# meuleman/epilogos

Measured on NVIDIA B200. Metric: bins/sec for expected+scores (S2), higher is better.
Workload: dtype int64+f64

## Files before the change

### epilogos_b200/csrc/common.cuh

```cuda
#pragma once
#include <cuda_runtime.h>
#include <cuda.h>
#include <stddef.h>
#include <stdint.h>
#include <stdio.h>
#include <string.h>

#include "../../include/epilogos_b200.h"

namespace epi {

void set_error(const char* fmt, ...);
int check_device();

#define EPI_CUDA(call)                                                                        \
    do {                                                                                      \
        cudaError_t e__ = (call);                                                             \
        if (e__ != cudaSuccess) {                                                             \
            epi::set_error("%s failed at %s:%d: %s", #call, __FILE__, __LINE__,               \
                           cudaGetErrorString(e__));                                          \
            return 1;                                                                         \
        }                                                                                     \
    } while (0)

#define EPI_REQUIRE(cond, ...)                                                                \
    do {                                                                                      \
        if (!(cond)) {                                                                        \
            epi::set_error(__VA_ARGS__);                                                      \
            return 2;                                                                         \
        }                                                                                     \
    } while (0)

int sm_count();
int persistent_grid(int64_t ntiles, int per_sm);

constexpr int S1_TABLE_MAX_WIDTH = 4095;

struct PrepFlags {
    int has_zero;
};

struct K5TcConsts {
    double dg[EPI_MAX_STATES];
    double scale;
    double cst;
    int has_zero;
    uint32_t m1, m8, m16;
    int fbits;
};

struct DeviceWorkspace {
    unsigned long long reduce_slots[64];
    double log2e[EPI_MAX_STATES * EPI_MAX_STATES];
    PrepFlags prep_flags;
    int s3_symmetric;
    alignas(16) uint8_t k5tc_b_image[8 * EPI_MAX_STATES * 128];
    K5TcConsts k5tc_consts;
    alignas(8) double s1_v64[EPI_MAX_STATES * (S1_TABLE_MAX_WIDTH + 1)];
    alignas(8) float s1_v32[EPI_MAX_STATES * (S1_TABLE_MAX_WIDTH + 1)];
    alignas(8) float perm_v32[2][EPI_MAX_STATES * (S1_TABLE_MAX_WIDTH + 1)];
};
static_assert(offsetof(DeviceWorkspace, k5tc_b_image) % 16 == 0, "the B operand image is a bulk-copy source");
static_assert(offsetof(DeviceWorkspace, s1_v64) % 8 == 0 && offsetof(DeviceWorkspace, s1_v32) % 8 == 0,
              "the S1 value tables need 8-byte alignment");

DeviceWorkspace* device_workspace();

typedef CUresult (*tensor_map_encode_fn)(CUtensorMap*, CUtensorMapDataType, cuuint32_t, void*, const cuuint64_t*,
                                         const cuuint64_t*, const cuuint32_t*, const cuuint32_t*,
                                         CUtensorMapInterleave, CUtensorMapSwizzle, CUtensorMapL2promotion,
                                         CUtensorMapFloatOOBfill);
tensor_map_encode_fn get_tensor_map_encode();

int s1_value_table(const float* e, int K, int width, float* v32, double* v64, cudaStream_t st);

int launch_k2_tc(const uint16_t* cnt, int64_t bins, int K, int64_t* n1, int64_t* n2, cudaStream_t st);
int scores_s2_tc(const uint16_t* cnt, int64_t bins, int K, int width, int64_t perms, const float* e, int* zero_flag,
                 float* o32, double* o64, cudaStream_t st);
bool scores_s2_tc_eligible(int width);
int scores_s2_tc_fixed_point(const float* e, int K, int64_t perms, unsigned long long* mfix_dev, int* fbits_host,
                             cudaStream_t st);

#ifdef __CUDACC__

__device__ __forceinline__ uint32_t smem_u32(const void* p) {
    return static_cast<uint32_t>(__cvta_generic_to_shared(p));
}

__device__ __forceinline__ void mbar_init(uint64_t* bar, uint32_t count) {
    asm volatile("mbarrier.init.shared::cta.b64 [%0], %1;" ::"r"(smem_u32(bar)), "r"(count));
}
__device__ __forceinline__ void mbar_fence_init() {
    asm volatile("fence.mbarrier_init.release.cluster;" ::: "memory");
}
__device__ __forceinline__ void mbar_expect_tx(uint64_t* bar, uint32_t bytes) {
    asm volatile("mbarrier.arrive.expect_tx.shared::cta.b64 _, [%0], %1;" ::"r"(smem_u32(bar)), "r"(bytes)
                 : "memory");
}
__device__ __forceinline__ void mbar_arrive(uint64_t* bar) {
    asm volatile("mbarrier.arrive.shared::cta.b64 _, [%0];" ::"r"(smem_u32(bar)) : "memory");
}
__device__ __forceinline__ void mbar_arrive_after(uint64_t* bar, uint32_t dep) {
    asm volatile("mbarrier.arrive.shared::cta.b64 _, [%0];" ::"r"(smem_u32(bar)), "r"(dep) : "memory");
}
__device__ __forceinline__ void mbar_arrive_after(uint64_t* bar, double dep) {
    asm volatile("mbarrier.arrive.shared::cta.b64 _, [%0];" ::"r"(smem_u32(bar)), "d"(dep) : "memory");
}
__device__ __forceinline__ bool mbar_try_wait(uint64_t* bar, uint32_t parity) {
    uint32_t ok;
    asm volatile(
        "{\n\t.reg .pred p;\n\t"
        "mbarrier.try_wait.parity.shared::cta.b64 p, [%1], %2;\n\t"
        "selp.u32 %0, 1, 0, p;\n\t}"
        : "=r"(ok)
        : "r"(smem_u32(bar)), "r"(parity)
        : "memory");
    return ok != 0;
}
__device__ __forceinline__ void mbar_wait(uint64_t* bar, uint32_t parity) {
    while (!mbar_try_wait(bar, parity)) {
    }
}

__device__ __forceinline__ void tma_load_2d(void* smem_dst, const CUtensorMap* map, int32_t c0, int32_t c1,
                                            uint64_t* bar) {
    asm volatile(
        "cp.async.bulk.tensor.2d.shared::cluster.global.tile.mbarrier::complete_tx::bytes [%0], [%1, {%2, %3}], [%4];"
        ::"r"(smem_u32(smem_dst)), "l"(reinterpret_cast<uint64_t>(map)), "r"(c0), "r"(c1), "r"(smem_u32(bar))
        : "memory");
}
__device__ __forceinline__ void bulk_load_1d(void* smem_dst, const void* gsrc, uint32_t bytes, uint64_t* bar) {
    asm volatile("cp.async.bulk.shared::cluster.global.mbarrier::complete_tx::bytes [%0], [%1], %2, [%3];"
                 ::"r"(smem_u32(smem_dst)), "l"(reinterpret_cast<uint64_t>(gsrc)), "r"(bytes), "r"(smem_u32(bar))
                 : "memory");
}
__device__ __forceinline__ void tma_prefetch_desc(const CUtensorMap* map) {
// ... 49 lines not shown
```

### epilogos_b200/csrc/scores.cu

```cuda
#include "common.cuh"

namespace epi {

constexpr int K5_THREADS = 256;
constexpr int K5_WARPS = K5_THREADS / 32;
constexpr int KT_MAX = EPI_MAX_STATES;

__constant__ __align__(16) double c_log2e[KT_MAX * KT_MAX];

__global__ void k5_prepare_kernel(const float* __restrict__ e, int rows, int cols, int kt, double* __restrict__ out,
                                  PrepFlags* flags) {
    __shared__ int zero;
    if (threadIdx.x == 0) zero = 0;
    __syncthreads();
    for (int i = threadIdx.x; i < rows * kt; i += blockDim.x) {
        const int s = i / kt, q = i - s * kt;
        double v = 0.0;
        if (q < cols) {
            const double ev = (double)e[s * cols + q];
            if (ev > 0.0) v = log2(ev);
            else zero = 1;
        }
        out[i] = v;
    }
    __syncthreads();
    if (threadIdx.x == 0) flags->has_zero = zero;
}

__device__ __forceinline__ double kl_direct(double obs, double e) {
    if (e == 0.0 || obs == 0.0) return 0.0;
    return obs * log2(obs / e);
}

struct WarpCountStream {
    const uint16_t* cnt;
    uint16_t* slab[2];
    uint64_t* bar;
    long long bins, ngroups, stride;
    int K, lane, buf;
    uint32_t phase[2];

    __device__ __forceinline__ void issue(long long g, int b) const {
        if (lane == 0 && g < ngroups && bins - g * 32 >= 32) {
            mbar_expect_tx(&bar[b], 64 * K);
            bulk_load_1d(slab[b], cnt + g * 32 * K, 64 * K, &bar[b]);
        }
    }
    __device__ __forceinline__ const uint16_t* acquire(long long g, int nvalid) {
        const int b = buf;
        buf ^= 1;
        issue(g + stride, b ^ 1);
        if (nvalid == 32) {
            mbar_wait(&bar[b], phase[b]);
            phase[b] ^= 1;
        } else {
            const uint16_t* src = cnt + g * 32 * K;
            for (int i = lane; i < nvalid * K; i += 32) slab[b][i] = src[i];
            __syncwarp();
        }
        return slab[b];
    }
};

__device__ __forceinline__ void warp_store_scores(const float* slab, float* __restrict__ dst, int nvalid, int K,
                                                  int lane) {
    __syncwarp();
    if (nvalid == 32) {
        const float4* s4 = reinterpret_cast<const float4*>(slab);
        float4* d4 = reinterpret_cast<float4*>(dst);
        for (int i = lane; i < 8 * K; i += 32) d4[i] = s4[i];
    } else {
        for (int i = lane; i < nvalid * K; i += 32) dst[i] = slab[i];
    }
    __syncwarp();
}

constexpr int S1_SMEM_TABLE_BYTES = 96 * 1024;

__global__ void k5_s1_table_kernel(const float* __restrict__ exp1, int K, int width, float* __restrict__ v32,
                                   double* __restrict__ v64) {
    const int n = K * (width + 1);
    const double dw = (double)width;
    for (int i = blockIdx.x * blockDim.x + threadIdx.x; i < n; i += gridDim.x * blockDim.x) {
        const int s = i / (width + 1), c = i - s * (width + 1);
// ... 16 lines not shown
    float* vts = reinterpret_cast<float*>(bars + K5_WARPS * 2);

    const int tid = threadIdx.x, warp = tid >> 5, lane = tid & 31;
    const int w1 = width + 1;
    if (tid == 0) {
        for (int i = 0; i < K5_WARPS * 2; ++i) mbar_init(&bars[i], 1);
        mbar_fence_init();
    }
    if (SMEM_TABLE)
        for (int i = tid; i < K * w1; i += K5_THREADS) vts[i] = v32g[i];
    __syncthreads();
    const float* vt = SMEM_TABLE ? vts : v32g;
    float* myf = fslab + warp * 32 * K;

    const long long ngroups = (bins + 31) / 32;
    WarpCountStream in{cnt, {cslab + warp * 64 * K, cslab + warp * 64 * K + 32 * K}, bars + warp * 2, bins, ngroups,
                       (long long)gridDim.x * K5_WARPS, K, lane, 0, {0u, 0u}};
    in.issue((long long)blockIdx.x * K5_WARPS + warp, 0);
    for (long long g = (long long)blockIdx.x * K5_WARPS + warp; g < ngroups; g += in.stride) {
        const long long bin0 = g * 32;
        const int nvalid = (int)((bins - bin0) < 32 ? (bins - bin0) : 32);
        const uint16_t* myc = in.acquire(g, nvalid);
        if (lane < nvalid) {
            const uint16_t* row = myc + lane * K;
            for (int s = 0; s < K; ++s) {
                const int c = row[s];
                myf[lane * K + s] = vt[s * w1 + c];
                if (out64 != nullptr) out64[(bin0 + lane) * K + s] = v64g[s * w1 + c];
            }
        }
        if (out32 != nullptr) warp_store_scores(myf, out32 + bin0 * K, nvalid, K, lane);
        else __syncwarp();
    }
}

__global__ void __launch_bounds__(K5_THREADS) k5_s1_direct_kernel(const uint16_t* __restrict__ cnt, long long bins, int K,
                                                                  int width, const float* __restrict__ exp1,
                                                                  float* __restrict__ out32, double* __restrict__ out64) {
    const double dw = (double)width;
    const long long n = bins * K;
    for (long long i = blockIdx.x * (long long)blockDim.x + threadIdx.x; i < n; i += (long long)gridDim.x * blockDim.x) {
        const int s = (int)(i % K);
        const double v = kl_direct((double)cnt[i] / dw, (double)__ldg(exp1 + s));
        if (out32 != nullptr) out32[i] = (float)v;
        if (out64 != nullptr) out64[i] = v;
    }
}

template <int KT>
__global__ void __launch_bounds__(K5_THREADS) k5_s2_kernel(const uint16_t* __restrict__ cnt, long long bins, int K,
                                                           int width, double perms, const float* __restrict__ exp2,
                                                           const PrepFlags* __restrict__ flags, int force_direct,
                                                           float* __restrict__ out32, double* __restrict__ out64) {
    if (force_direct == 2 && !flags->has_zero) return;
    extern __shared__ __align__(128) uint8_t smem_raw[];
    uint16_t* cslab = reinterpret_cast<uint16_t*>(smem_raw);
    float* fslab = reinterpret_cast<float*>(smem_raw + K5_WARPS * 32 * K * 4);
    uint64_t* bars = reinterpret_cast<uint64_t*>(smem_raw + K5_WARPS * 32 * K * 8);

    const int tid = threadIdx.x, warp = tid >> 5, lane = tid & 31;
    if (tid == 0) {
        for (int i = 0; i < K5_WARPS * 2; ++i) mbar_init(&bars[i], 1);
        mbar_fence_init();
    }
    __syncthreads();
    const double lp = log2(perms);
    const double inv_perms = 1.0 / perms;
    const bool direct = force_direct || flags->has_zero;
    float* myf = fslab + warp * 32 * K;

    const long long ngroups = (bins + 31) / 32;
    WarpCountStream in{cnt, {cslab + warp * 64 * K, cslab + warp * 64 * K + 32 * K}, bars + warp * 2, bins, ngroups,
                       (long long)gridDim.x * K5_WARPS, K, lane, 0, {0u, 0u}};
    in.issue((long long)blockIdx.x * K5_WARPS + warp, 0);
    for (long long g = (long long)blockIdx.x * K5_WARPS + warp; g < ngroups; g += in.stride) {
        const long long bin0 = g * 32;
        const int nvalid = (int)((bins - bin0) < 32 ? (bins - bin0) : 32);
        const uint16_t* myc = in.acquire(g, nvalid);
        if (lane < nvalid) {
            const uint16_t* row = myc + lane * K;
            float* orow = myf + lane * K;
            if (direct) {
                for (int q = 0; q < K; ++q) {
                    const long long cq = row[q];
                    double sum = 0.0;
                    if (cq != 0) {
                        for (int s = 0; s < K; ++s) {
                            const long long cs = row[s];
                            const long long prod = (s == q) ? cs * (cs - 1) : cs * cq;
                            if (prod != 0) sum += kl_direct((double)prod / perms, (double)__ldg(exp2 + s * K + q));
                        }
                    }
                    orow[q] = (float)sum;
                    if (out64 != nullptr) out64[(bin0 + lane) * K + q] = sum;
                }
            } else {
                double cd[KT], mc[KT];
                double a = 0.0, w = 0.0;
#pragma unroll
                for (int s = 0; s < KT; ++s) {
                    const int c = s < K ? row[s] : 0;
                    cd[s] = (double)c;
                    const double l = c > 0 ? log2((double)c) : 0.0;
                    a = fma(cd[s], l, a);
                    w += cd[s];
                    mc[s] = 0.0;
                }
                const double2* le2 = reinterpret_cast<const double2*>(c_log2e);
#pragma unroll
                for (int s = 0; s < KT; ++s) {
#pragma unroll
                    for (int q = 0; q < KT; q += 2) {
                        const double2 m = le2[(s * KT + q) >> 1];
                        mc[q] = fma(cd[s], m.x, mc[q]);
                        mc[q + 1] = fma(cd[s], m.y, mc[q + 1]);
                    }
                }
                const double wm1 = w - 1.0;
#pragma unroll
                for (int q = 0; q < KT; ++q) {
                    if (q < K) {
                        const int c = row[q];
                        const int cm = c > 0 ? c - 1 : 0;
                        const double lt = c > 0 ? log2((double)c) : 0.0;
                        const double l1 = cm > 0 ? log2((double)cm) : 0.0;
                        double br = (a - mc[q]) + c_log2e[q * KT + q];
                        br = fma(lt - lp, wm1, br);
                        br = fma(-cd[q], lt, br);
                        br = fma((double)cm, l1, br);
                        const double v = c > 0 ? (cd[q] * inv_perms) * br : 0.0;
                        orow[q] = (float)v;
                        if (out64 != nullptr) out64[(bin0 + lane) * K + q] = v;
                    }
                }
            }
        }
        if (out32 != nullptr) warp_store_scores(myf, out32 + bin0 * K, nvalid, K, lane);
        else __syncwarp();
    }
}

static int prepare_tables(const float* e, int rows, int cols, int kt, cudaStream_t st, const PrepFlags** flags_out) {
    DeviceWorkspace* ws = device_workspace();
    EPI_REQUIRE(ws != nullptr, "could not allocate the per-device workspace");
    k5_prepare_kernel<<<1, 256, 0, st>>>(e, rows, cols, kt, ws->log2e, &ws->prep_flags);
// ... 17 lines not shown
        const int64_t cap = (int64_t)sm_count() * 16;
        if (blocks > cap) blocks = cap;
        k5_s1_direct_kernel<<<(unsigned)blocks, K5_THREADS, 0, st>>>(cnt, bins, K, width, e, o32, o64);
        EPI_CUDA(cudaGetLastError());
        return 0;
    }
    DeviceWorkspace* ws = device_workspace();
    EPI_REQUIRE(ws != nullptr, "could not allocate the per-device workspace");
    double* v64 = ws->s1_v64;
    float* v32 = ws->s1_v32;
    const int n = K * (width + 1);
    if (int rc = s1_value_table(e, K, width, v32, v64, st)) return rc;
    const size_t base = (size_t)K5_WARPS * 32 * K * 8 + K5_WARPS * 16;
    const size_t table = (size_t)n * 4;
    const int64_t ntiles = (bins + K5_THREADS - 1) / K5_THREADS;
    const size_t base_big = (size_t)32 * 32 * K * 8 + 32 * 16;
    if (table <= (size_t)S1_SMEM_TABLE_BYTES && 4 * (base + table + 1024) > (size_t)220 * 1024 &&
        base_big + table + 1024 <= (size_t)226 * 1024) {
        auto kern = k5_s1_kernel<true, 1024>;
        EPI_CUDA(cudaFuncSetAttribute(kern, cudaFuncAttributeMaxDynamicSharedMemorySize, (int)(base_big + table)));
        kern<<<persistent_grid((bins + 1023) / 1024, 1), 1024, base_big + table, st>>>(cnt, bins, K, width, v32, v64, o32, o64);
    } else if (table <= (size_t)S1_SMEM_TABLE_BYTES) {
        auto kern = k5_s1_kernel<true, K5_THREADS>;
        EPI_CUDA(cudaFuncSetAttribute(kern, cudaFuncAttributeMaxDynamicSharedMemorySize, (int)(base + table)));
        const int per_sm = (int)((size_t)220 * 1024 / (base + table + 1024));
        kern<<<persistent_grid(ntiles, per_sm < 1 ? 1 : (per_sm > 4 ? 4 : per_sm)), K5_THREADS, base + table, st>>>(
            cnt, bins, K, width, v32, v64, o32, o64);
    } else {
        auto kern = k5_s1_kernel<false, K5_THREADS>;
        EPI_CUDA(cudaFuncSetAttribute(kern, cudaFuncAttributeMaxDynamicSharedMemorySize, (int)base));
        kern<<<persistent_grid(ntiles, 4), K5_THREADS, base, st>>>(cnt, bins, K, width, v32, v64, o32, o64);
    }
    EPI_CUDA(cudaGetLastError());
    return 0;
}

template <int KT>
static int launch_s2(const uint16_t* cnt, int64_t bins, int K, int width, int64_t perms, const float* e,
                     const PrepFlags* flags, int direct, float* o32, double* o64, cudaStream_t st) {
    auto kern = k5_s2_kernel<KT>;
    const size_t smem = (size_t)K5_WARPS * 32 * K * 8 + K5_WARPS * 16;
    EPI_CUDA(cudaFuncSetAttribute(kern, cudaFuncAttributeMaxDynamicSharedMemorySize, (int)smem));
    const int64_t ntiles = (bins + K5_THREADS - 1) / K5_THREADS;
    kern<<<persistent_grid(ntiles, 3), K5_THREADS, smem, st>>>(cnt, bins, K, width, (double)perms, e, flags, direct, o32,
                                                                o64);
    EPI_CUDA(cudaGetLastError());
    return 0;
}

template <int KT>
static int dispatch_s2(const uint16_t* cnt, int64_t bins, int K, int width, int64_t perms, const float* e, float* o32,
                       double* o64, int mode, cudaStream_t st) {
    const PrepFlags* flags = nullptr;
    if (mode == EPI_SCORE_TABLE && scores_s2_tc_eligible(width)) {
        DeviceWorkspace* ws = device_workspace();
        EPI_REQUIRE(ws != nullptr, "could not allocate the per-device workspace");
        PrepFlags* fl = &ws->prep_flags;
        if (int rc = scores_s2_tc(cnt, bins, K, width, perms, e, &fl->has_zero, o32, o64, st)) return rc;
        return launch_s2<KT>(cnt, bins, K, width, perms, e, fl, 2, o32, o64, st);
    }
    if (int rc = prepare_tables(e, K, K, KT, st, &flags)) return rc;
    return launch_s2<KT>(cnt, bins, K, width, perms, e, flags, mode == EPI_SCORE_DIRECT, o32, o64, st);
}

}

using namespace epi;

static int check_score_args(const void* cnt, int64_t bins, int K, int width, const void* e, int mode) {
    if (check_device()) return 3;
    EPI_REQUIRE(bins >= 0 && bins < (1ll << 31), "bins=%lld out of range", (long long)bins);
    EPI_REQUIRE(K >= 1 && K <= EPI_MAX_STATES, "num_states=%d out of range [1, %d]", K, EPI_MAX_STATES);
    EPI_REQUIRE(width >= 1 && width <= 65535, "width=%d out of range [1, 65535]", width);
    EPI_REQUIRE(mode == EPI_SCORE_TABLE || mode == EPI_SCORE_DIRECT, "unknown score mode %d", mode);
    if (bins == 0) return 0;
    EPI_REQUIRE(cnt != nullptr && e != nullptr, "null pointer argument");
    EPI_REQUIRE((reinterpret_cast<uintptr_t>(cnt) & 15) == 0, "cnt_dev must be 16-byte aligned");
    return 0;
}

extern "C" int epi_scores_s1(const uint16_t* cnt_dev, int64_t bins, int32_t K, int32_t width, const float* exp1_dev,
                             float* out32_dev, double* out64_dev, int32_t mode, void* stream_) {
    cudaStream_t st = static_cast<cudaStream_t>(stream_);
    if (int rc = check_score_args(cnt_dev, bins, K, width, exp1_dev, mode)) return rc;
    if (bins == 0 || (out32_dev == nullptr && out64_dev == nullptr)) return 0;
    EPI_REQUIRE(out32_dev == nullptr || (reinterpret_cast<uintptr_t>(out32_dev) & 15) == 0,
                "out32_dev must be 16-byte aligned");
    return launch_s1(cnt_dev, bins, K, width, exp1_dev, mode == EPI_SCORE_DIRECT, out32_dev, out64_dev, st);
}

extern "C" int epi_scores_s2_fixed_point(const float* exp2_dev, int32_t K, int64_t perms, uint64_t* mfix_dev,
                                         int32_t* fraction_bits_out, void* stream_) {
    cudaStream_t st = static_cast<cudaStream_t>(stream_);
    if (check_device()) return 3;
    EPI_REQUIRE(K >= 1 && K <= EPI_MAX_STATES, "num_states=%d out of range [1, %d]", K, EPI_MAX_STATES);
    EPI_REQUIRE(perms >= 1 && exp2_dev != nullptr && mfix_dev != nullptr, "bad argument");
    int fbits = 0;
    if (int rc = scores_s2_tc_fixed_point(exp2_dev, K, perms, reinterpret_cast<unsigned long long*>(mfix_dev), &fbits, st))
        return rc;
    if (fraction_bits_out) *fraction_bits_out = fbits;
    return 0;
}

extern "C" int epi_scores_s2(const uint16_t* cnt_dev, int64_t bins, int32_t K, int32_t width, int64_t perms,
                             const float* exp2_dev, float* out32_dev, double* out64_dev, int32_t mode, void* stream_) {
    cudaStream_t st = static_cast<cudaStream_t>(stream_);
    if (int rc = check_score_args(cnt_dev, bins, K, width, exp2_dev, mode)) return rc;
    EPI_REQUIRE(perms >= 1, "perms=%lld must be positive (needs at least 2 biosamples)", (long long)perms);
    if (bins == 0 || (out32_dev == nullptr && out64_dev == nullptr)) return 0;
    EPI_REQUIRE(out32_dev == nullptr || (reinterpret_cast<uintptr_t>(out32_dev) & 15) == 0,
                "out32_dev must be 16-byte aligned");
    if (K <= 16) return dispatch_s2<16>(cnt_dev, bins, K, width, perms, exp2_dev, out32_dev, out64_dev, mode, st);
    if (K <= 18) return dispatch_s2<18>(cnt_dev, bins, K, width, perms, exp2_dev, out32_dev, out64_dev, mode, st);
// ... 3 lines not shown
```

### epilogos_b200/csrc/tc_tables.cu

```cuda
#include "common.cuh"
#include "tc05.cuh"
#include "count_tile.cuh"

namespace epi {

constexpr int T2_BINS = 128;
constexpr int T2_STAGES = 4;
constexpr int T2_OPS = 2;
constexpr int T2_THREADS = 192;
constexpr int T2_TMEM_COLS = 128;

template <int KT, int KR>
__global__ void __launch_bounds__(T2_THREADS, 4)
k2_tc_kernel(const uint16_t* __restrict__ cnt, long long bins, int Krt, unsigned long long* __restrict__ n1,
             unsigned long long* __restrict__ n2) {
    const int K = KR ? KR : Krt;
    constexpr int NCOL = ((2 * KT + 1) + 15) & ~15;
    extern __shared__ uint8_t smem_raw[];
    uint8_t* smem = smem_raw + ((1024u - (smem_u32(smem_raw) & 1023u)) & 1023u);
    const int tile_bytes = T2_BINS * K * 2;
    uint8_t* ops = smem;
    uint8_t* ring = ops + T2_OPS * T2_OP_BYTES;
    uint64_t* ld_full = reinterpret_cast<uint64_t*>(ring + T2_STAGES * tile_bytes);
    uint64_t* ld_empty = ld_full + T2_STAGES;
// ... 96 lines not shown
                    drain_gram<NCOL>(tmem_base + ((uint32_t)(warp * 32) << 16), warp, lane, K, n1, n2);
                    tc_fence_before();
                    __syncwarp();
                    if (lane == 0) mbar_arrive(acc_empty);
                }
            }
        }
    }
    tc_fence_before();
    __syncthreads();
    if (warp == 5) tmem_dealloc(tmem_base, T2_TMEM_COLS);
}

template <int KT, int KR>
static int launch_k2_tc_impl(const uint16_t* cnt, int64_t bins, int K, int64_t* n1, int64_t* n2, cudaStream_t st) {
    const size_t smem = 1024 + (size_t)T2_OPS * T2_OP_BYTES + (size_t)T2_STAGES * T2_BINS * K * 2 +
                        (2 * T2_STAGES + 2 * T2_OPS + 2) * 8 + 16;
    auto kern = k2_tc_kernel<KT, KR>;
    EPI_CUDA(cudaFuncSetAttribute(kern, cudaFuncAttributeMaxDynamicSharedMemorySize, (int)smem));
    const int64_t ntiles = (bins + T2_BINS - 1) / T2_BINS;
    const int ctas = 4;
    kern<<<persistent_grid(ntiles, ctas), T2_THREADS, smem, st>>>(cnt, (long long)bins, K,
                                                                reinterpret_cast<unsigned long long*>(n1),
                                                                reinterpret_cast<unsigned long long*>(n2));
    EPI_CUDA(cudaGetLastError());
    return 0;
}

int launch_k2_tc(const uint16_t* cnt, int64_t bins, int K, int64_t* n1, int64_t* n2, cudaStream_t st) {
    if (K == 18) return launch_k2_tc_impl<18, 18>(cnt, bins, K, n1, n2, st);
    if (K == 15) return launch_k2_tc_impl<16, 15>(cnt, bins, K, n1, n2, st);
    if (K <= 16) return launch_k2_tc_impl<16, 0>(cnt, bins, K, n1, n2, st);
    if (K <= 18) return launch_k2_tc_impl<18, 0>(cnt, bins, K, n1, n2, st);
    return launch_k2_tc_impl<32, 0>(cnt, bins, K, n1, n2, st);
}

constexpr int T5_BINS = 128;
constexpr int T5_A_BYTES = 128 * 128;
constexpr unsigned long long T5_MAGIC = 0x4338000000000000ull;
constexpr int T5_MAX_WIDTH = 2047;

__device__ __forceinline__ unsigned long long mad_wide(uint32_t a, uint32_t b, unsigned long long c) {
    unsigned long long d;
    asm("mad.wide.u32 %0, %1, %2, %3;" : "=l"(d) : "r"(a), "r"(b), "l"(c));
    return d;
}

__device__ __forceinline__ uint32_t mad_lo(uint32_t a, uint32_t b, uint32_t c) {
    uint32_t d;
    asm("mad.lo.u32 %0, %1, %2, %3;" : "=r"(d) : "r"(a), "r"(b), "r"(c));
    return d;
}

__constant__ K5TcConsts c_k5tc;

__global__ void k5tc_prepare_kernel(const float* __restrict__ e, int K, double perms, int nrows,
                                    uint8_t* __restrict__ b_image, K5TcConsts* __restrict__ out, int* __restrict__ zero_flag,
                                    unsigned long long* __restrict__ mfix_out) {
    __shared__ unsigned long long mfix[EPI_MAX_STATES * EPI_MAX_STATES];
    __shared__ double mval[EPI_MAX_STATES * EPI_MAX_STATES];
    __shared__ unsigned long long maxbits;
    __shared__ int zero, fbits;
    if (threadIdx.x == 0) {
        maxbits = 0ull;
        zero = 0;
    }
    __syncthreads();
    for (int i = threadIdx.x; i < K * K; i += blockDim.x) {
        const double ev = (double)e[i];
        double m = 0.0;
        if (ev > 0.0) m = -log2(ev);
        else zero = 1;
        if (m < 0.0) m = 0.0;
        mval[i] = m;
        atomicMax(&maxbits, (unsigned long long)__double_as_longlong(m));
    }
    __syncthreads();
    if (threadIdx.x == 0) {
        const double mx = __longlong_as_double((long long)maxbits);
        int ib = 1;
        while (ib < 12 && (double)(1ull << ib) <= mx) ++ib;
        fbits = 56 - ib;
    }
    __syncthreads();
    const int F = fbits;
    for (int i = threadIdx.x; i < K * K; i += blockDim.x) {
        unsigned long long v = (unsigned long long)llrint(ldexp(mval[i], F));
        if (v >= (1ull << 56)) v = (1ull << 56) - 1;
        mfix[i] = v;
        if (mfix_out != nullptr) mfix_out[i] = v;
    }
    for (int i = threadIdx.x; i < nrows * 128 / 4; i += blockDim.x) reinterpret_cast<uint32_t*>(b_image)[i] = 0u;
    __syncthreads();
    for (int i = threadIdx.x; i < K * K * 14; i += blockDim.x) {
        const int dd = i % 7, h = (i / 7) & 1, st = i / 14;
        const int s = st / K, t = st - s * K;
        const uint32_t n = (uint32_t)(t * 8 + dd + h), k = (uint32_t)(2 * s + h);
        b_image[sw128_offset(n, k)] = (uint8_t)((mfix[st] >> (8 * dd)) & 255ull);
    }
    if (threadIdx.x < K) out->dg[threadIdx.x] = ldexp((double)mfix[threadIdx.x * K + threadIdx.x], -F - 3) / perms;
    if (threadIdx.x == 0) {
        const double scale = ldexp(1.0, -F) / perms;
        out->scale = scale;
        out->cst = 6755399441055744.0 * scale;
        out->has_zero = zero;
        out->m1 = 1u;
        out->m8 = 1u << 8;
        out->m16 = 1u << 16;
        out->fbits = F;
        *zero_flag = zero;
    }
}

template <int KT, int KR, int NWG, bool WANT64>
__global__ void __launch_bounds__(NWG * 128 + 64, 1)
k5_s2_tc_kernel(const uint16_t* __restrict__ cnt, long long bins, int Krt, int width, double perms,
                const uint8_t* __restrict__ b_image, float* __restrict__ out32, double* __restrict__ out64) {
    if (c_k5tc.has_zero) return;

    static_assert(KT % 2 == 0, "KT must be even");
    constexpr int NPAD = ((8 * KT + 31) / 32) * 32;
    static_assert(NPAD * NWG <= 512, "accumulator regions exceed TMEM");
    constexpr int KSTEPS = (2 * KT + 31) / 32;
    const int K = KR ? KR : Krt;

    extern __shared__ uint8_t smem_raw[];
    uint8_t* smem = smem_raw + ((1024u - (smem_u32(smem_raw) & 1023u)) & 1023u);
    const int slab_bytes = T5_BINS * K * 2;
    uint8_t* a_ops = smem;
    uint8_t* b_op = a_ops + NWG * T5_A_BYTES;
    uint8_t* slabs = b_op + NPAD * 128;
    float* stage = reinterpret_cast<float*>(slabs + NWG * 2 * slab_bytes);
    double* g1 = reinterpret_cast<double*>(stage + NWG * T5_BINS * K);
    double* f1 = g1 + ((width + 2) & ~1);
    uint64_t* ld_full = reinterpret_cast<uint64_t*>(f1 + ((width + 2) & ~1));
    uint64_t* ld_empty = ld_full + NWG * 2;
    uint64_t* a_full = ld_empty + NWG * 2;
    uint64_t* mma_done = a_full + NWG;
    uint64_t* b_full = mma_done + NWG;
    uint32_t* tmem_slot = reinterpret_cast<uint32_t*>(b_full + 1);

    const int tid = threadIdx.x, warp = tid >> 5, lane = tid & 31;
    constexpr int NT = NWG * 128 + 64;
    const long long ntiles = (bins + T5_BINS - 1) / T5_BINS;
    const long long nfull = bins / T5_BINS;

    for (int i = tid; i < NWG * T5_A_BYTES / 16; i += NT) reinterpret_cast<uint4*>(a_ops)[i] = make_uint4(0u, 0u, 0u, 0u);
    {
        const double lp = log2(perms), invp = 1.0 / perms, wm1 = (double)width - 1.0;
        for (int c = tid; c <= width; c += NT) {
            const double l = c > 0 ? log2((double)c) : 0.0;
            const double l1 = c > 1 ? log2((double)(c - 1)) : 0.0;
            const double cl = (double)c * l;
            f1[c] = cl * invp;
            g1[c] = (double)c * ((fma(l - lp, wm1, -cl) + (double)(c > 0 ? c - 1 : 0) * l1) * invp);
        }
    }
    fence_proxy_async_smem();
    if (tid == 0) {
        for (int i = 0; i < NWG * 2; ++i) {
            mbar_init(&ld_full[i], 1);
            mbar_init(&ld_empty[i], 4);
        }
        for (int g = 0; g < NWG; ++g) {
            mbar_init(&a_full[g], 4);
            mbar_init(&mma_done[g], 1);
        }
        mbar_init(b_full, 1);
        mbar_fence_init();
    }
    if (warp == 4 * NWG + 1) tmem_alloc(tmem_slot, 512);
    tc_fence_before();
    __syncthreads();
    tc_fence_after();
    const uint32_t tmem_base = *tmem_slot;

    if (warp == 4 * NWG) {
        if (lane == 0) {
            mbar_expect_tx(b_full, NPAD * 128);
            bulk_load_1d(b_op, b_image, NPAD * 128, b_full);
            int j = 0;
            for (long long t = blockIdx.x; t < nfull; t += gridDim.x, ++j) {
                const int g = j % NWG, u = j / NWG, b = u & 1;
                mbar_wait_wd(&ld_empty[g * 2 + b], (((uint32_t)(u >> 1)) & 1u) ^ 1u);
                mbar_expect_tx(&ld_full[g * 2 + b], (uint32_t)slab_bytes);
                bulk_load_1d(slabs + (g * 2 + b) * slab_bytes, cnt + t * (long long)T5_BINS * K, (uint32_t)slab_bytes,
                             &ld_full[g * 2 + b]);
            }
        }
    } else if (warp == 4 * NWG + 1) {
        if (lane == 0) {
            const uint32_t nmma = (uint32_t)((8 * K + 15) & ~15);
            const uint32_t idesc = umma_i8_idesc(128, nmma);
            mbar_wait_wd(b_full, 0);
            const uint64_t b_desc = make_kmajor_sw128_desc(smem_u32(b_op));
            int j = 0;
            for (long long t = blockIdx.x; t < ntiles; t += gridDim.x, ++j) {
                const int g = j % NWG, u = j / NWG;
                mbar_wait_spin_wd(&a_full[g], ((uint32_t)u) & 1u);
                tc_fence_after();
                const uint64_t a_desc = make_kmajor_sw128_desc(smem_u32(a_ops + g * T5_A_BYTES));
#pragma unroll
                for (int k = 0; k < KSTEPS; ++k)
                    umma_i8(tmem_base + (uint32_t)(g * NPAD), a_desc + 2 * k, b_desc + 2 * k, idesc, k ? 1u : 0u);
                umma_commit(&mma_done[g]);
            }
        }
    } else {
        const int g = warp >> 2, r = tid & 127;
        uint8_t* a_row = a_ops + g * T5_A_BYTES + r * 128;
        float* mystage = stage + g * T5_BINS * K;
        const uint32_t taddr = tmem_base + ((uint32_t)((warp & 3) * 32) << 16) + (uint32_t)(g * NPAD);
        const double scale = c_k5tc.scale * 0.125, cst = c_k5tc.cst, scale32 = c_k5tc.scale * (4294967296.0 * 0.125);
        int u = 0;
        for (long long t = blockIdx.x + (long long)g * gridDim.x; t < ntiles; t += (long long)NWG * gridDim.x, ++u) {
            const long long bin0 = t * T5_BINS;
            const int b = u & 1;
            uint32_t cw[KT / 2];
            if (t < nfull) {
                mbar_wait_wd(&ld_full[g * 2 + b], ((uint32_t)(u >> 1)) & 1u);
                load_count_row<KT, KR>(reinterpret_cast<const uint16_t*>(slabs + (g * 2 + b) * slab_bytes) + r * K, K, cw);
            } else {
                load_count_row_guarded<KT>(cnt + (bin0 + r) * K, K, bin0 + r < bins, cw);
            }
            store_operand_row<KT>(a_row, r, cw, -1, 0u);
            fence_proxy_async_smem();
            __syncwarp();
            if (lane == 0) {
                mbar_arrive(&a_full[g]);
                if (t < nfull) mbar_arrive(&ld_empty[g * 2 + b]);
            }

            uint32_t co[KT];
#pragma unroll
            for (int s = 0; s < KT; ++s) co[s] = ((cw[s >> 1] >> (16 * (s & 1))) & 0xffffu) << 3;
            double a4[4] = {0.0, 0.0, 0.0, 0.0};
#pragma unroll
            for (int s = 0; s < KT; ++s) a4[s & 3] += *reinterpret_cast<const double*>(reinterpret_cast<const uint8_t*>(f1) + co[s]);
            const double a_adj = (((a4[0] + a4[1]) + (a4[2] + a4[3])) - cst) * 0.125;

            if (lane == 0) bulk_wait_read0();
            __syncwarp();
            mbar_wait_wd(&mma_done[g], ((uint32_t)u) & 1u);
            tc_fence_after();
#pragma unroll
            for (int c0 = 0; c0 < 8 * KT; c0 += 32) {
                uint32_t v[32];
                double chg[4], cd[4];
#pragma unroll
                for (int i = 0; i < 4; ++i) {
                    const int tt = (c0 / 8 + i < KT) ? c0 / 8 + i : 0;
                    chg[i] = *reinterpret_cast<const double*>(reinterpret_cast<const uint8_t*>(g1) + co[tt]);
                    cd[i] = __hiloint2double(0x43300000, (int)co[tt]) - 4503599627370496.0;
                }
                tmem_ld_32x32(taddr + (uint32_t)c0, v);
                float f[4];
#pragma unroll
                for (int i = 0; i < 4; ++i) {
                    const int tt = c0 / 8 + i;
                    f[i] = 0.0f;
                    if (tt < KT && (KR == 0 || tt < KR)) {
                        const uint32_t t01 = mad_lo(v[8 * i + 1], c_k5tc.m8, v[8 * i]);
                        const uint32_t t23 = mad_lo(v[8 * i + 3], c_k5tc.m8, v[8 * i + 2]);
                        const uint32_t t45 = mad_lo(v[8 * i + 5], c_k5tc.m8, v[8 * i + 4]);
                        const uint32_t t67 = mad_lo(v[8 * i + 7], c_k5tc.m8, v[8 * i + 6]);
                        const unsigned long long lb = mad_wide(t23, c_k5tc.m16, ((unsigned long long)(T5_MAGIC >> 32) << 32) | t01);
                        const unsigned long long hb = mad_wide(t67, c_k5tc.m16, ((unsigned long long)(T5_MAGIC >> 32) << 32) | t45);
                        const double dl = __longlong_as_double((long long)lb);
                        const double dh = __longlong_as_double((long long)hb) - 6755399441055744.0;
                        const double base = fma(dh, scale32, fma(dl, scale, a_adj)) - c_k5tc.dg[tt];
                        const double val = fma(cd[i], base, chg[i]);
                        f[i] = (float)val;
                        if (WANT64 && (KR != 0 || tt < K) && bin0 + r < bins) out64[(bin0 + r) * K + tt] = val;
                    }
                }
                if constexpr (KR != 0 && KR % 2 == 0) {
                    float2* dst = reinterpret_cast<float2*>(mystage + r * KR + c0 / 8);
                    if (c0 / 8 < KR) dst[0] = make_float2(f[0], f[1]);
                    if (c0 / 8 + 2 < KR) dst[1] = make_float2(f[2], f[3]);
                } else {
#pragma unroll
                    for (int i = 0; i < 4; ++i)
                        if (c0 / 8 + i < K) mystage[r * K + c0 / 8 + i] = f[i];
                }
            }
            tc_fence_before();
            fence_proxy_async_smem();
            __syncwarp();
            if (out32 != nullptr) {
                const int wq = warp & 3;
                const long long wbin0 = bin0 + 32 * wq;
                if (t < nfull) {
                    if (lane == 0) {
                        bulk_store_1d(out32 + wbin0 * K, mystage + 32 * wq * K, (uint32_t)(32 * K * 4));
                        bulk_commit();
                    }
                } else if (wbin0 < bins) {
                    const int n = (int)((bins - wbin0) < 32 ? (bins - wbin0) : 32) * K;
                    for (int i = lane; i < n; i += 32) out32[wbin0 * K + i] = mystage[32 * wq * K + i];
                }
            }
        }
        if (lane == 0) bulk_wait0();
    }
    tc_fence_before();
    __syncthreads();
    if (warp == 4 * NWG + 1) tmem_dealloc(tmem_base, 512);
}

template <int KT, int KR, int NWG, bool WANT64>
static int launch_k5_tc2(const uint16_t* cnt, int64_t bins, int K, int width, int64_t perms, const uint8_t* b_image,
                         float* o32, double* o64, cudaStream_t st) {
    constexpr int NPAD = ((8 * KT + 31) / 32) * 32;
    auto kern = k5_s2_tc_kernel<KT, KR, NWG, WANT64>;
    const size_t smem = 1024 + (size_t)NWG * T5_A_BYTES + (size_t)NPAD * 128 + (size_t)NWG * 2 * T5_BINS * K * 2 +
                        (size_t)NWG * T5_BINS * K * 4 + (size_t)(width + 2) * 16 +
                        (size_t)(6 * NWG + 1) * 8 + 16;
    EPI_CUDA(cudaFuncSetAttribute(kern, cudaFuncAttributeMaxDynamicSharedMemorySize, (int)smem));
    const int64_t ntiles = (bins + T5_BINS - 1) / T5_BINS;
    kern<<<persistent_grid(ntiles, 1), NWG * 128 + 64, smem, st>>>(cnt, (long long)bins, K, width, (double)perms, b_image,
                                                                    o32, o64);
    EPI_CUDA(cudaGetLastError());
    return 0;
}

template <int KT, int KR, int NWG>
static int launch_k5_tc(const uint16_t* cnt, int64_t bins, int K, int width, int64_t perms, const float* e, int* zero_flag,
                        float* o32, double* o64, cudaStream_t st) {
    constexpr int NPAD = ((8 * KT + 31) / 32) * 32;
    static_assert(NPAD * 128 <= sizeof(DeviceWorkspace::k5tc_b_image), "B operand image exceeds its workspace region");
    DeviceWorkspace* ws = device_workspace();
    EPI_REQUIRE(ws != nullptr, "could not allocate the per-device workspace");
    k5tc_prepare_kernel<<<1, 256, 0, st>>>(e, K, (double)perms, NPAD, ws->k5tc_b_image, &ws->k5tc_consts, zero_flag, nullptr);
    EPI_CUDA(cudaGetLastError());
    EPI_CUDA(cudaMemcpyToSymbolAsync(c_k5tc, &ws->k5tc_consts, sizeof(K5TcConsts), 0, cudaMemcpyDeviceToDevice, st));
    if (o64 != nullptr) return launch_k5_tc2<KT, KR, NWG, true>(cnt, bins, K, width, perms, ws->k5tc_b_image, o32, o64, st);
    return launch_k5_tc2<KT, KR, NWG, false>(cnt, bins, K, width, perms, ws->k5tc_b_image, o32, o64, st);
}

int scores_s2_tc(const uint16_t* cnt, int64_t bins, int K, int width, int64_t perms, const float* e, int* zero_flag,
                 float* o32, double* o64, cudaStream_t st) {
    if (K == 18) return launch_k5_tc<18, 18, 3>(cnt, bins, K, width, perms, e, zero_flag, o32, o64, st);
    if (K == 15) return launch_k5_tc<16, 15, 4>(cnt, bins, K, width, perms, e, zero_flag, o32, o64, st);
    if (K <= 16) return launch_k5_tc<16, 0, 4>(cnt, bins, K, width, perms, e, zero_flag, o32, o64, st);
    if (K <= 18) return launch_k5_tc<18, 0, 3>(cnt, bins, K, width, perms, e, zero_flag, o32, o64, st);
    return launch_k5_tc<32, 0, 2>(cnt, bins, K, width, perms, e, zero_flag, o32, o64, st);
}

bool scores_s2_tc_eligible(int width) { return width <= T5_MAX_WIDTH; }

int scores_s2_tc_fixed_point(const float* e, int K, int64_t perms, unsigned long long* mfix_dev, int* fbits_host,
                             cudaStream_t st) {
    DeviceWorkspace* ws = device_workspace();
    EPI_REQUIRE(ws != nullptr, "could not allocate the per-device workspace");
    k5tc_prepare_kernel<<<1, 256, 0, st>>>(e, K, (double)perms, 8 * EPI_MAX_STATES, ws->k5tc_b_image, &ws->k5tc_consts,
                                           &ws->prep_flags.has_zero, mfix_dev);
    EPI_CUDA(cudaGetLastError());
    K5TcConsts host;
    EPI_CUDA(cudaMemcpyAsync(&host, &ws->k5tc_consts, sizeof(host), cudaMemcpyDeviceToHost, st));
    EPI_CUDA(cudaStreamSynchronize(st));
    if (fbits_host) *fbits_host = host.fbits;
    return 0;
}

}
```

Measured before the change: 5.263 billion.

## Fold zero-fallback into TC kernel, decouple TMEM accumulators from warpgroups

Removes the constant-memory copy and the separate fallback launch: the TC scoring kernel now reads the constants through a pointer and handles the has-zero case itself with an inline direct-score loop. TMEM accumulator regions are decoupled from warpgroups through NACC slots guarded by acc_empty barriers. This allows K=18 to run 4 warpgroups with 3 accumulators. The intent is fewer launches and memcpys per call and more epilogue warpgroups for K in 17–18, at the cost of extra barrier waits, and the MMA can stall until an accumulator is freed.

Measured after the change: 5.351 billion, median of 6. +1.7%, better.

```diff
diff --git a/epilogos_b200/csrc/common.cuh b/epilogos_b200/csrc/common.cuh
--- a/epilogos_b200/csrc/common.cuh
+++ b/epilogos_b200/csrc/common.cuh
@@ -45,7 +45,6 @@
     double scale;
     double cst;
     int has_zero;
-    uint32_t m1, m8, m16;
     int fbits;
 };
 
@@ -75,13 +74,31 @@
 int s1_value_table(const float* e, int K, int width, float* v32, double* v64, cudaStream_t st);
 
 int launch_k2_tc(const uint16_t* cnt, int64_t bins, int K, int64_t* n1, int64_t* n2, cudaStream_t st);
-int scores_s2_tc(const uint16_t* cnt, int64_t bins, int K, int width, int64_t perms, const float* e, int* zero_flag,
-                 float* o32, double* o64, cudaStream_t st);
+int scores_s2_tc(const uint16_t* cnt, int64_t bins, int K, int width, int64_t perms, const float* e, float* o32,
+                 double* o64, cudaStream_t st);
 bool scores_s2_tc_eligible(int width);
 int scores_s2_tc_fixed_point(const float* e, int K, int64_t perms, unsigned long long* mfix_dev, int* fbits_host,
                              cudaStream_t st);
 
 #ifdef __CUDACC__
+
+__device__ __forceinline__ double kl_direct(double obs, double e) {
+    if (e == 0.0 || obs == 0.0) return 0.0;
+    return obs * log2(obs / e);
+}
+__device__ __forceinline__ double s2_direct_score(const uint16_t* row, int K, int q, double perms,
+                                                  const float* __restrict__ exp2) {
+    const long long cq = row[q];
+    double sum = 0.0;
+    if (cq != 0) {
+        for (int s = 0; s < K; ++s) {
+            const long long cs = row[s];
+            const long long prod = (s == q) ? cs * (cs - 1) : cs * cq;
+            if (prod != 0) sum += kl_direct((double)prod / perms, (double)__ldg(exp2 + s * K + q));
+        }
+    }
+    return sum;
+}
 
 __device__ __forceinline__ uint32_t smem_u32(const void* p) {
     return static_cast<uint32_t>(__cvta_generic_to_shared(p));
diff --git a/epilogos_b200/csrc/scores.cu b/epilogos_b200/csrc/scores.cu
--- a/epilogos_b200/csrc/scores.cu
+++ b/epilogos_b200/csrc/scores.cu
@@ -25,11 +25,6 @@
     }
     __syncthreads();
     if (threadIdx.x == 0) flags->has_zero = zero;
-}
-
-__device__ __forceinline__ double kl_direct(double obs, double e) {
-    if (e == 0.0 || obs == 0.0) return 0.0;
-    return obs * log2(obs / e);
 }
 
 struct WarpCountStream {
@@ -152,7 +147,6 @@
                                                            int width, double perms, const float* __restrict__ exp2,
                                                            const PrepFlags* __restrict__ flags, int force_direct,
                                                            float* __restrict__ out32, double* __restrict__ out64) {
-    if (force_direct == 2 && !flags->has_zero) return;
     extern __shared__ __align__(128) uint8_t smem_raw[];
     uint16_t* cslab = reinterpret_cast<uint16_t*>(smem_raw);
     float* fslab = reinterpret_cast<float*>(smem_raw + K5_WARPS * 32 * K * 4);
@@ -182,15 +176,7 @@
             float* orow = myf + lane * K;
             if (direct) {
                 for (int q = 0; q < K; ++q) {
-                    const long long cq = row[q];
-                    double sum = 0.0;
-                    if (cq != 0) {
-                        for (int s = 0; s < K; ++s) {
-                            const long long cs = row[s];
-                            const long long prod = (s == q) ? cs * (cs - 1) : cs * cq;
-                            if (prod != 0) sum += kl_direct((double)prod / perms, (double)__ldg(exp2 + s * K + q));
-                        }
-                    }
+                    const double sum = s2_direct_score(row, K, q, perms, exp2);
                     orow[q] = (float)sum;
                     if (out64 != nullptr) out64[(bin0 + lane) * K + q] = sum;
                 }
@@ -314,13 +300,8 @@
 static int dispatch_s2(const uint16_t* cnt, int64_t bins, int K, int width, int64_t perms, const float* e, float* o32,
                        double* o64, int mode, cudaStream_t st) {
     const PrepFlags* flags = nullptr;
-    if (mode == EPI_SCORE_TABLE && scores_s2_tc_eligible(width)) {
-        DeviceWorkspace* ws = device_workspace();
-        EPI_REQUIRE(ws != nullptr, "could not allocate the per-device workspace");
-        PrepFlags* fl = &ws->prep_flags;
-        if (int rc = scores_s2_tc(cnt, bins, K, width, perms, e, &fl->has_zero, o32, o64, st)) return rc;
-        return launch_s2<KT>(cnt, bins, K, width, perms, e, fl, 2, o32, o64, st);
-    }
+    if (mode == EPI_SCORE_TABLE && scores_s2_tc_eligible(width))
+        return scores_s2_tc(cnt, bins, K, width, perms, e, o32, o64, st);
     if (int rc = prepare_tables(e, K, K, KT, st, &flags)) return rc;
     return launch_s2<KT>(cnt, bins, K, width, perms, e, flags, mode == EPI_SCORE_DIRECT, o32, o64, st);
 }
diff --git a/epilogos_b200/csrc/tc_tables.cu b/epilogos_b200/csrc/tc_tables.cu
--- a/epilogos_b200/csrc/tc_tables.cu
+++ b/epilogos_b200/csrc/tc_tables.cu
@@ -172,10 +172,10 @@
     return d;
 }
 
-__constant__ K5TcConsts c_k5tc;
+__constant__ uint32_t c_m8 = 1u << 8, c_m16 = 1u << 16;
 
 __global__ void k5tc_prepare_kernel(const float* __restrict__ e, int K, double perms, int nrows,
-                                    uint8_t* __restrict__ b_image, K5TcConsts* __restrict__ out, int* __restrict__ zero_flag,
+                                    uint8_t* __restrict__ b_image, K5TcConsts* __restrict__ out,
                                     unsigned long long* __restrict__ mfix_out) {
     __shared__ unsigned long long mfix[EPI_MAX_STATES * EPI_MAX_STATES];
     __shared__ double mval[EPI_MAX_STATES * EPI_MAX_STATES];
@@ -218,33 +218,44 @@
         const uint32_t n = (uint32_t)(t * 8 + dd + h), k = (uint32_t)(2 * s + h);
         b_image[sw128_offset(n, k)] = (uint8_t)((mfix[st] >> (8 * dd)) & 255ull);
     }
-    if (threadIdx.x < K) out->dg[threadIdx.x] = ldexp((double)mfix[threadIdx.x * K + threadIdx.x], -F - 3) / perms;
+    if (threadIdx.x < EPI_MAX_STATES)
+        out->dg[threadIdx.x] = threadIdx.x < K ? ldexp((double)mfix[threadIdx.x * K + threadIdx.x], -F - 3) / perms : 0.0;
     if (threadIdx.x == 0) {
         const double scale = ldexp(1.0, -F) / perms;
         out->scale = scale;
         out->cst = 6755399441055744.0 * scale;
         out->has_zero = zero;
-        out->m1 = 1u;
-        out->m8 = 1u << 8;
-        out->m16 = 1u << 16;
         out->fbits = F;
-        *zero_flag = zero;
-    }
-}
-
-template <int KT, int KR, int NWG, bool WANT64>
+    }
+}
+
+template <int KT, int KR, int NWG, int NACC, bool WANT64>
 __global__ void __launch_bounds__(NWG * 128 + 64, 1)
 k5_s2_tc_kernel(const uint16_t* __restrict__ cnt, long long bins, int Krt, int width, double perms,
-                const uint8_t* __restrict__ b_image, float* __restrict__ out32, double* __restrict__ out64) {
-    if (c_k5tc.has_zero) return;
-
+                const uint8_t* __restrict__ b_image, const K5TcConsts* __restrict__ kc, const float* __restrict__ exp2,
+                float* __restrict__ out32, double* __restrict__ out64) {
     static_assert(KT % 2 == 0, "KT must be even");
     constexpr int NPAD = ((8 * KT + 31) / 32) * 32;
-    static_assert(NPAD * NWG <= 512, "accumulator regions exceed TMEM");
+    static_assert(NPAD * NACC <= 512, "accumulator regions exceed TMEM");
+    static_assert(NACC <= NWG, "more accumulator regions than warpgroups to fill them");
     constexpr int KSTEPS = (2 * KT + 31) / 32;
+    constexpr int NT = NWG * 128 + 64;
     const int K = KR ? KR : Krt;
+    const int tid = threadIdx.x, warp = tid >> 5, lane = tid & 31;
+
+    if (kc->has_zero) {
+        const long long n = bins * K;
+        for (long long i = (long long)blockIdx.x * NT + tid; i < n; i += (long long)gridDim.x * NT) {
+            const long long b = i / K;
+            const double v = s2_direct_score(cnt + b * K, K, (int)(i - b * K), perms, exp2);
+            if (out32 != nullptr) out32[i] = (float)v;
+            if (WANT64) out64[i] = v;
+        }
+        return;
+    }
 
     extern __shared__ uint8_t smem_raw[];
+    __shared__ __align__(16) double s_dg[EPI_MAX_STATES];
     uint8_t* smem = smem_raw + ((1024u - (smem_u32(smem_raw) & 1023u)) & 1023u);
     const int slab_bytes = T5_BINS * K * 2;
     uint8_t* a_ops = smem;
@@ -257,15 +268,15 @@
     uint64_t* ld_empty = ld_full + NWG * 2;
     uint64_t* a_full = ld_empty + NWG * 2;
     uint64_t* mma_done = a_full + NWG;
-    uint64_t* b_full = mma_done + NWG;
+    uint64_t* acc_empty = mma_done + NWG;
+    uint64_t* b_full = acc_empty + NACC;
     uint32_t* tmem_slot = reinterpret_cast<uint32_t*>(b_full + 1);
 
-    const int tid = threadIdx.x, warp = tid >> 5, lane = tid & 31;
-    constexpr int NT = NWG * 128 + 64;
     const long long ntiles = (bins + T5_BINS - 1) / T5_BINS;
     const long long nfull = bins / T5_BINS;
 
     for (int i = tid; i < NWG * T5_A_BYTES / 16; i += NT) reinterpret_cast<uint4*>(a_ops)[i] = make_uint4(0u, 0u, 0u, 0u);
+    if (tid < EPI_MAX_STATES) s_dg[tid] = kc->dg[tid];
     {
         const double lp = log2(perms), invp = 1.0 / perms, wm1 = (double)width - 1.0;
         for (int c = tid; c <= width; c += NT) {
@@ -286,6 +297,7 @@
             mbar_init(&a_full[g], 4);
             mbar_init(&mma_done[g], 1);
         }
+        for (int q = 0; q < NACC; ++q) mbar_init(&acc_empty[q], 4);
         mbar_init(b_full, 1);
         mbar_fence_init();
     }
@@ -316,13 +328,14 @@
             const uint64_t b_desc = make_kmajor_sw128_desc(smem_u32(b_op));
             int j = 0;
             for (long long t = blockIdx.x; t < ntiles; t += gridDim.x, ++j) {
-                const int g = j % NWG, u = j / NWG;
+                const int g = j % NWG, u = j / NWG, q = j % NACC, n = j / NACC;
+                mbar_wait_spin_wd(&acc_empty[q], (((uint32_t)n) & 1u) ^ 1u);
                 mbar_wait_spin_wd(&a_full[g], ((uint32_t)u) & 1u);
                 tc_fence_after();
                 const uint64_t a_desc = make_kmajor_sw128_desc(smem_u32(a_ops + g * T5_A_BYTES));
 #pragma unroll
                 for (int k = 0; k < KSTEPS; ++k)
-                    umma_i8(tmem_base + (uint32_t)(g * NPAD), a_desc + 2 * k, b_desc + 2 * k, idesc, k ? 1u : 0u);
+                    umma_i8(tmem_base + (uint32_t)(q * NPAD), a_desc + 2 * k, b_desc + 2 * k, idesc, k ? 1u : 0u);
                 umma_commit(&mma_done[g]);
             }
         }
@@ -330,12 +343,13 @@
         const int g = warp >> 2, r = tid & 127;
         uint8_t* a_row = a_ops + g * T5_A_BYTES + r * 128;
         float* mystage = stage + g * T5_BINS * K;
-        const uint32_t taddr = tmem_base + ((uint32_t)((warp & 3) * 32) << 16) + (uint32_t)(g * NPAD);
-        const double scale = c_k5tc.scale * 0.125, cst = c_k5tc.cst, scale32 = c_k5tc.scale * (4294967296.0 * 0.125);
+        const uint32_t tlane = tmem_base + ((uint32_t)((warp & 3) * 32) << 16);
+        const double scale = kc->scale * 0.125, cst = kc->cst, scale32 = kc->scale * (4294967296.0 * 0.125);
         int u = 0;
         for (long long t = blockIdx.x + (long long)g * gridDim.x; t < ntiles; t += (long long)NWG * gridDim.x, ++u) {
             const long long bin0 = t * T5_BINS;
             const int b = u & 1;
+            const int q = (u * NWG + g) % NACC;
             uint32_t cw[KT / 2];
             if (t < nfull) {
                 mbar_wait_wd(&ld_full[g * 2 + b], ((uint32_t)(u >> 1)) & 1u);
@@ -363,6 +377,7 @@
             __syncwarp();
             mbar_wait_wd(&mma_done[g], ((uint32_t)u) & 1u);
             tc_fence_after();
+            const uint32_t taddr = tlane + (uint32_t)(q * NPAD);
 #pragma unroll
             for (int c0 = 0; c0 < 8 * KT; c0 += 32) {
                 uint32_t v[32];
@@ -373,6 +388,9 @@
                     chg[i] = *reinterpret_cast<const double*>(reinterpret_cast<const uint8_t*>(g1) + co[tt]);
                     cd[i] = __hiloint2double(0x43300000, (int)co[tt]) - 4503599627370496.0;
                 }
+                const double2 dg01 = *reinterpret_cast<const double2*>(s_dg + c0 / 8);
+                const double2 dg23 = *reinterpret_cast<const double2*>(s_dg + c0 / 8 + 2);
+                const double dg[4] = {dg01.x, dg01.y, dg23.x, dg23.y};
                 tmem_ld_32x32(taddr + (uint32_t)c0, v);
                 float f[4];
 #pragma unroll
@@ -380,15 +398,15 @@
                     const int tt = c0 / 8 + i;
                     f[i] = 0.0f;
                     if (tt < KT && (KR == 0 || tt < KR)) {
-                        const uint32_t t01 = mad_lo(v[8 * i + 1], c_k5tc.m8, v[8 * i]);
-                        const uint32_t t23 = mad_lo(v[8 * i + 3], c_k5tc.m8, v[8 * i + 2]);
-                        const uint32_t t45 = mad_lo(v[8 * i + 5], c_k5tc.m8, v[8 * i + 4]);
-                        const uint32_t t67 = mad_lo(v[8 * i + 7], c_k5tc.m8, v[8 * i + 6]);
-                        const unsigned long long lb = mad_wide(t23, c_k5tc.m16, ((unsigned long long)(T5_MAGIC >> 32) << 32) | t01);
-                        const unsigned long long hb = mad_wide(t67, c_k5tc.m16, ((unsigned long long)(T5_MAGIC >> 32) << 32) | t45);
+                        const uint32_t t01 = mad_lo(v[8 * i + 1], c_m8, v[8 * i]);
+                        const uint32_t t23 = mad_lo(v[8 * i + 3], c_m8, v[8 * i + 2]);
+                        const uint32_t t45 = mad_lo(v[8 * i + 5], c_m8, v[8 * i + 4]);
+                        const uint32_t t67 = mad_lo(v[8 * i + 7], c_m8, v[8 * i + 6]);
+                        const unsigned long long lb = mad_wide(t23, c_m16, ((unsigned long long)(T5_MAGIC >> 32) << 32) | t01);
+                        const unsigned long long hb = mad_wide(t67, c_m16, ((unsigned long long)(T5_MAGIC >> 32) << 32) | t45);
                         const double dl = __longlong_as_double((long long)lb);
                         const double dh = __longlong_as_double((long long)hb) - 6755399441055744.0;
-                        const double base = fma(dh, scale32, fma(dl, scale, a_adj)) - c_k5tc.dg[tt];
+                        const double base = fma(dh, scale32, fma(dl, scale, a_adj)) - dg[i];
                         const double val = fma(cd[i], base, chg[i]);
                         f[i] = (float)val;
                         if (WANT64 && (KR != 0 || tt < K) && bin0 + r < bins) out64[(bin0 + r) * K + tt] = val;
@@ -407,6 +425,7 @@
             tc_fence_before();
             fence_proxy_async_smem();
             __syncwarp();
+            if (lane == 0) mbar_arrive(&acc_empty[q]);
             if (out32 != nullptr) {
                 const int wq = warp & 3;
                 const long long wbin0 = bin0 + 32 * wq;
@@ -428,43 +447,45 @@
     if (warp == 4 * NWG + 1) tmem_dealloc(tmem_base, 512);
 }
 
-template <int KT, int KR, int NWG, bool WANT64>
+template <int KT, int KR, int NWG, int NACC, bool WANT64>
 static int launch_k5_tc2(const uint16_t* cnt, int64_t bins, int K, int width, int64_t perms, const uint8_t* b_image,
-                         float* o32, double* o64, cudaStream_t st) {
+                         const K5TcConsts* kc, const float* e, float* o32, double* o64, cudaStream_t st) {
     constexpr int NPAD = ((8 * KT + 31) / 32) * 32;
-    auto kern = k5_s2_tc_kernel<KT, KR, NWG, WANT64>;
+    auto kern = k5_s2_tc_kernel<KT, KR, NWG, NACC, WANT64>;
     const size_t smem = 1024 + (size_t)NWG * T5_A_BYTES + (size_t)NPAD * 128 + (size_t)NWG * 2 * T5_BINS * K * 2 +
                         (size_t)NWG * T5_BINS * K * 4 + (size_t)(width + 2) * 16 +
-                        (size_t)(6 * NWG + 1) * 8 + 16;
+                        (size_t)(6 * NWG + NACC + 1) * 8 + 16;
     EPI_CUDA(cudaFuncSetAttribute(kern, cudaFuncAttributeMaxDynamicSharedMemorySize, (int)smem));
     const int64_t ntiles = (bins + T5_BINS - 1) / T5_BINS;
     kern<<<persistent_grid(ntiles, 1), NWG * 128 + 64, smem, st>>>(cnt, (long long)bins, K, width, (double)perms, b_image,
-                                                                    o32, o64);
+                                                                    kc, e, o32, o64);
     EPI_CUDA(cudaGetLastError());
     return 0;
 }
 
-template <int KT, int KR, int NWG>
-static int launch_k5_tc(const uint16_t* cnt, int64_t bins, int K, int width, int64_t perms, const float* e, int* zero_flag,
-                        float* o32, double* o64, cudaStream_t st) {
+template <int KT, int KR, int NWG, int NACC>
+static int launch_k5_tc(const uint16_t* cnt, int64_t bins, int K, int width, int64_t perms, const float* e, float* o32,
+                        double* o64, cudaStream_t st) {
     constexpr int NPAD = ((8 * KT + 31) / 32) * 32;
     static_assert(NPAD * 128 <= sizeof(DeviceWorkspace::k5tc_b_image), "B operand image exceeds its workspace region");
     DeviceWorkspace* ws = device_workspace();
     EPI_REQUIRE(ws != nullptr, "could not allocate the per-device workspace");
-    k5tc_prepare_kernel<<<1, 256, 0, st>>>(e, K, (double)perms, NPAD, ws->k5tc_b_image, &ws->k5tc_consts, zero_flag, nullptr);
+    k5tc_prepare_kernel<<<1, 256, 0, st>>>(e, K, (double)perms, NPAD, ws->k5tc_b_image, &ws->k5tc_consts, nullptr);
     EPI_CUDA(cudaGetLastError());
-    EPI_CUDA(cudaMemcpyToSymbolAsync(c_k5tc, &ws->k5tc_consts, sizeof(K5TcConsts), 0, cudaMemcpyDeviceToDevice, st));
-    if (o64 != nullptr) return launch_k5_tc2<KT, KR, NWG, true>(cnt, bins, K, width, perms, ws->k5tc_b_image, o32, o64, st);
-    return launch_k5_tc2<KT, KR, NWG, false>(cnt, bins, K, width, perms, ws->k5tc_b_image, o32, o64, st);
-}
-
-int scores_s2_tc(const uint16_t* cnt, int64_t bins, int K, int width, int64_t perms, const float* e, int* zero_flag,
-                 float* o32, double* o64, cudaStream_t st) {
-    if (K == 18) return launch_k5_tc<18, 18, 3>(cnt, bins, K, width, perms, e, zero_flag, o32, o64, st);
-    if (K == 15) return launch_k5_tc<16, 15, 4>(cnt, bins, K, width, perms, e, zero_flag, o32, o64, st);
-    if (K <= 16) return launch_k5_tc<16, 0, 4>(cnt, bins, K, width, perms, e, zero_flag, o32, o64, st);
-    if (K <= 18) return launch_k5_tc<18, 0, 3>(cnt, bins, K, width, perms, e, zero_flag, o32, o64, st);
-    return launch_k5_tc<32, 0, 2>(cnt, bins, K, width, perms, e, zero_flag, o32, o64, st);
+    if (o64 != nullptr)
+        return launch_k5_tc2<KT, KR, NWG, NACC, true>(cnt, bins, K, width, perms, ws->k5tc_b_image, &ws->k5tc_consts, e,
+                                                      o32, o64, st);
+    return launch_k5_tc2<KT, KR, NWG, NACC, false>(cnt, bins, K, width, perms, ws->k5tc_b_image, &ws->k5tc_consts, e, o32,
+                                                   o64, st);
+}
+
+int scores_s2_tc(const uint16_t* cnt, int64_t bins, int K, int width, int64_t perms, const float* e, float* o32,
+                 double* o64, cudaStream_t st) {
+    if (K == 18) return launch_k5_tc<18, 18, 4, 3>(cnt, bins, K, width, perms, e, o32, o64, st);
+    if (K == 15) return launch_k5_tc<16, 15, 4, 4>(cnt, bins, K, width, perms, e, o32, o64, st);
+    if (K <= 16) return launch_k5_tc<16, 0, 4, 4>(cnt, bins, K, width, perms, e, o32, o64, st);
+    if (K <= 18) return launch_k5_tc<18, 0, 4, 3>(cnt, bins, K, width, perms, e, o32, o64, st);
+    return launch_k5_tc<32, 0, 2, 2>(cnt, bins, K, width, perms, e, o32, o64, st);
 }
 
 bool scores_s2_tc_eligible(int width) { return width <= T5_MAX_WIDTH; }
@@ -474,7 +495,7 @@
     DeviceWorkspace* ws = device_workspace();
     EPI_REQUIRE(ws != nullptr, "could not allocate the per-device workspace");
     k5tc_prepare_kernel<<<1, 256, 0, st>>>(e, K, (double)perms, 8 * EPI_MAX_STATES, ws->k5tc_b_image, &ws->k5tc_consts,
-                                           &ws->prep_flags.has_zero, mfix_dev);
+                                           mfix_dev);
     EPI_CUDA(cudaGetLastError());
     K5TcConsts host;
     EPI_CUDA(cudaMemcpyAsync(&host, &ws->k5tc_consts, sizeof(host), cudaMemcpyDeviceToHost, st));
```
